# etrigger/Parsip

Measured on AMD Instinct MI355X. Metric: Mcells/sec polygonized, 256^3 grid 32-prim BlobTree, at 1/2/4/8 MI355X, higher is better.
Workload: dtype f32

## Files before the change

parsip_amd/csrc/psgpu_device.h:

```cpp
#pragma once
#include "psgpu_model.h"

namespace psgpu {

typedef const __attribute__((address_space(4))) DevModel* ModelPtr;
typedef const __attribute__((address_space(4))) DevPrim CPrim;
typedef const __attribute__((address_space(4))) DevOp COp;
typedef const __attribute__((address_space(4))) CubeTablesDev* TablePtr;
__device__ __forceinline__ ModelPtr as_const(const DevModel* m) { return (ModelPtr)m; }
__device__ __forceinline__ TablePtr as_const(const CubeTablesDev* t) { return (TablePtr)t; }

__device__ __forceinline__ Instr load_instr(ModelPtr M, int pc) {
    typedef const __attribute__((address_space(4))) uint32_t* CU32;
    const CU32 w = (CU32)(&M->instr[pc]);
    const uint32_t words[3] = {w[0], w[1], w[2]};
    Instr I;
    __builtin_memcpy(&I, words, 12);
    return I;
}

__device__ __forceinline__ float max_ref(float a, float b) { return a > b ? a : b; }
__device__ __forceinline__ float min_ref(float a, float b) { return a < b ? a : b; }
__device__ __forceinline__ float m01(bool c) { return c ? 1.0f : 0.0f; }
__device__ __forceinline__ int lane_id() { return __lane_id(); }
// ... 539 lines not shown
    return (hw & 0xffffu) | (xcc << 16);
}
__device__ __forceinline__ void mpu_ticks_s1(const Params& p, uint32_t w, uint64_t t0) {
    uint64_t* r = p.mpuTicks + 4 * (size_t)w;
    r[0] = t0;
    r[1] = stamp_now();
    r[2] = 0ull;
    r[3] = (uint64_t)wave_hw_id();
}
__device__ __forceinline__ void mpu_ticks_s2(const Params& p, uint32_t m) {
    const uint64_t t = stamp_now();
    const uint32_t hw = wave_hw_id();
    if (lane_id() == 0) {
        uint64_t* r = p.mpuTicks + 4 * (size_t)(m - p.mpuBegin);
        atomicMax(reinterpret_cast<unsigned long long*>(r + 2), (unsigned long long)t);
        reinterpret_cast<uint32_t*>(r + 3)[1] = hw;
    }
}
#define PSGPU_STAMPED(K, ITEM, CALL)                                             \
    {                                                                             \
        const uint64_t t0_ = (p.stamps || p.spans) ? psgpu::stamp_now() : 0ull;  \
        uint32_t item_ = blockIdx.x * (blockDim.x >> 6) + (threadIdx.x >> 6);     \
        CALL;                                                                     \
        if (K == 1 && p.mpuTicks && ITEM != 0xffffffffu) psgpu::mpu_ticks_s2(p, ITEM); \
        if (p.stamps) psgpu::stamp_end(p, K, t0_, ITEM);                          \
        if (p.spans) psgpu::span_end(p, K, t0_);                                  \
    }

__device__ __forceinline__ void mpu_origin(const Params& p, uint32_t m, float o[3]) {
    uint32_t k, jk;
    const uint32_t i = div_by(m, p.dims[2] * p.dims[1], p.divMagic[1], &jk);
    const uint32_t j = div_by(jk, p.dims[2], p.divMagic[0], &k);
    o[0] = p.lo[0] + (float)i * p.side;
    o[1] = p.lo[1] + (float)j * p.side;
    o[2] = p.lo[2] + (float)k * p.side;
}

__device__ __forceinline__ uint32_t wave_sum(uint32_t v) { return lane_value(wave_incl_scan(v), 63); }


__device__ __forceinline__ uint32_t front_tag(const Params& p) { return p.ctr->epoch + 1u; }

__device__ __forceinline__ void stamp_live_word(const Params& p, bool on, const CullMask& cm, uint64_t above) {
    if (on && p.stamps && lane_id() == 0) {
        const uint32_t w = blockIdx.x * (blockDim.x >> 6) + (threadIdx.x >> 6);
        if (w < p.stampCap)
            p.stamps[3 * (size_t)kNumStampKernels * p.stampCap + 8 * (size_t)w + 7] =
                (uint64_t)(128 - __popcll(cm.lo) - __popcll(cm.hi)) | above;
    }
}

__device__ __forceinline__ BoundBox octant_box(const Params& p, const float o[3], int c) {
    BoundBox B;
#pragma unroll
    for (int i = 0; i < 4; ++i) {
        B.xs[i] = o[0] + (float)(4 * (c & 1) + i) * p.cs;
        B.ys[i] = o[1] + (float)(4 * ((c >> 1) & 1) + i) * p.cs;
        B.zs[i] = o[2] + (float)(4 * (c >> 2) + i) * p.cs;
    }
    const float hx = 0.5f * (B.xs[3] - B.xs[0]), hy = 0.5f * (B.ys[3] - B.ys[0]), hz = 0.5f * (B.zs[3] - B.zs[0]);
    B.cx = 0.5f * (B.xs[0] + B.xs[3]);
    B.cy = 0.5f * (B.ys[0] + B.ys[3]);
    B.cz = 0.5f * (B.zs[0] + B.zs[3]);
    B.h = __builtin_amdgcn_sqrtf(hx * hx + hy * hy + hz * hz) * 1.0001f + 1e-4f;
    float mag = 0.0f;
#pragma unroll
    for (int a = 0; a < 3; ++a)
        mag = fmaxf(mag, fmaxf(fabsf(p.lo[a]), fabsf(p.lo[a] + (float)p.dims[a] * p.side)));
    B.hx = B.hy = B.hz = (1.5f * p.cs + 2.4e-7f * (mag + p.side)) * 1.0001f + 1e-4f;
    return B;
}

__device__ __forceinline__ uint32_t proven_mask(bool ok, float lo, float hi, uint32_t flags8) {
    const uint64_t bOut = ballot(ok && hi < 0.5f), bIn = ballot(ok && lo >= 0.5f);
    uint32_t proven8 = 0;
#pragma unroll
    for (int q = 0; q < 8; ++q) {
        const bool all = ((bOut >> (8 * q)) & 0xffull) == 0xffull || ((bIn >> (8 * q)) & 0xffull) == 0xffull;
        proven8 |= (all ? 1u : 0u) << q;
    }
    return proven8 & flags8;
}

__device__ __forceinline__ CullMask queue_masks(const Params& p, const CullLanes& cl, const float o[3],
                                                uint32_t queue8, uint32_t mOf, int lane) {
    CullMask mine{0ull, 0ull};
    if (!p.cull) return mine;
    const float eg = 7.0f * p.cs + 0.001f;
    ModelPtr Mo = as_const(p.model);
    const uint32_t nOps = p.opInside ? Mo->ctOps : 0u;
    float bl[2][3], bh[2][3];
#pragma unroll
    for (int h = 0; h < 2; ++h) {
        const uint32_t k = 64u * h + (uint32_t)lane;
#pragma unroll
        for (int a = 0; a < 3; ++a) {
            bl[h][a] = k < nOps ? p.model->ops[k].lo[a] : 1.0f;
            bh[h][a] = k < nOps ? p.model->ops[k].hi[a] : -1.0f;
        }
    }
    for (uint32_t qm = queue8; qm != 0u; qm &= qm - 1u) {
        const int q = __builtin_ctz(qm);
        const float ox = __int_as_float(__builtin_amdgcn_readlane(__float_as_int(o[0]), 8 * q));
        const float oy = __int_as_float(__builtin_amdgcn_readlane(__float_as_int(o[1]), 8 * q));
        const float oz = __int_as_float(__builtin_amdgcn_readlane(__float_as_int(o[2]), 8 * q));
        CullMask g = cull_mask_from(cl, ox, oy, oz, ox + eg, oy + eg, oz + eg);
        if (nOps != 0u) g.inLo = ballot((uint32_t)lane < nOps && op_inside_box(bl[0], bh[0], ox, oy, oz, p.cs));
        if (nOps > 64u)
            g.inHi = ballot(64u + (uint32_t)lane < nOps && op_inside_box(bl[1], bh[1], ox, oy, oz, p.cs));
        const uint32_t wq = lane_value(mOf, q) - p.mpuBegin;
        if (lane == 0) {
            p.mpuMasks[4 * wq] = g.lo;
            p.mpuMasks[4 * wq + 1] = g.hi;
            p.mpuMasks[4 * wq + 2] = g.inLo;
            p.mpuMasks[4 * wq + 3] = g.inHi;
        }
        if (lane == q) mine = g;
    }
    return mine;
}

struct QueueEntry {
    uint32_t m;
    CullMask cm;

    template <bool FRONT, class T>
    static __device__ __forceinline__ void put(T* at, T v) {
        if constexpr (FRONT) __hip_atomic_store(at, v, __ATOMIC_RELAXED, __HIP_MEMORY_SCOPE_AGENT);
        else *at = v;
    }
    template <bool FRONT, class T>
    static __device__ __forceinline__ T get(T* at) {
        if constexpr (FRONT) return __hip_atomic_load(at, __ATOMIC_RELAXED, __HIP_MEMORY_SCOPE_AGENT);
        else return *at;
    }
    template <bool FRONT>
    __device__ __forceinline__ void store(const Params& p, uint32_t slotq) const {
        put<FRONT>(&p.pq[slotq], m);
        if (p.cull) {
            put<FRONT>(&p.pqMask[4 * slotq], cm.lo);
            put<FRONT>(&p.pqMask[4 * slotq + 1], cm.hi);
            put<FRONT>(&p.pqMask[4 * slotq + 2], cm.inLo);
            put<FRONT>(&p.pqMask[4 * slotq + 3], cm.inHi);
        }
    }
    static __device__ __forceinline__ void publish(const Params& p, uint32_t slotq, bool mine) {
        asm volatile("s_waitcnt vmcnt(0)" ::: "memory");
        if (mine) put<true>(&p.fqReady[slotq], front_tag(p));
    }
    template <bool FRONT>
    static __device__ __forceinline__ QueueEntry load(const Params& p, ModelPtr M, uint32_t slotq) {
        QueueEntry e{uniform(get<FRONT>(&p.pq[slotq])), CullMask{0ull, 0ull}};
        if (p.cull) {
            e.cm.lo = uniform64(get<FRONT>(&p.pqMask[4 * slotq]));
            e.cm.hi = uniform64(get<FRONT>(&p.pqMask[4 * slotq + 1]));
            e.cm.inLo = uniform64(get<FRONT>(&p.pqMask[4 * slotq + 2]));
            if (!FRONT || M->ctOps > 64u) e.cm.inHi = uniform64(get<FRONT>(&p.pqMask[4 * slotq + 3]));
        }
        return e;
    }
};

template <class EV, int SPLIT = 1, bool FRONT = false>
__device__ __forceinline__ void precheck_body(const Params& p, float* lds) {
    const int wave = (int)uniform((uint32_t)wave_index());
    const int lane = lane_id();
    const int part = wave % SPLIT;
    const int slot = wave / SPLIT;
    phase_stamp(p, 0, 8192u);
    const uint64_t tick0 = p.mpuTicks ? stamp_now() : 0ull;
    if (blockIdx.x == 0 && threadIdx.x == 0) {
        p.hostCtr->surfaceErr = 0u;
        p.totals[7] = 0u;
    }
    EV ev(as_const(p.model), lds + wave * p.slotsPerLane * 64 + lane);
    CullLanes cl;
    if (p.cull) cl = load_cull_lanes(as_const(p.model));
    const uint32_t W = blockIdx.x * (4u / SPLIT) + (uint32_t)slot;
    uint32_t Wq = W;
    if constexpr (SPLIT == 2) asm volatile("" : "+v"(Wq));
    const uint32_t bzN = p.brickDims[2], byN = p.brickDims[1];
    const uint32_t nBricks = p.brickDims[0] * byN * bzN;
    uint32_t bi, bj, bk;
    bool idle = W >= nBricks;
    if (p.sieve) {
        typedef const __attribute__((address_space(4))) uint64_t* CU64;
        typedef const __attribute__((address_space(4))) uint32_t* CU32;
        const uint64_t e = W < nBricks ? ((CU64)p.liveList)[W] : 0ull;
        idle = W >= *(CU32)&p.ctr->liveBricks;
        bi = (uint32_t)e & 0x1fffffu;
        bj = (uint32_t)(e >> 21) & 0x1fffffu;
        bk = (uint32_t)(e >> 42);
    } else {
        const uint32_t B =
            (idle || p.brickStride == 1u) ? W : (uint32_t)(((uint64_t)W * p.brickStride) % nBricks);
        uint32_t jk;
        bi = p.brickI0 + div_by(B, byN * bzN, p.brickMagic[1], &jk);
        bj = div_by(jk, bzN, p.brickMagic[0], &bk);
    }
    if (SPLIT == 1 && idle) return;
    const uint32_t g = (uint32_t)lane >> 3;
    const uint32_t mi = 2u * bi + ((g >> 2) & 1u);
    const uint32_t mj = 2u * bj + ((g >> 1) & 1u);
    const uint32_t mk = 2u * bk + (g & 1u);
    const uint32_t mg = (mi * p.dims[1] + mj) * p.dims[2] + mk;
    const bool valid = !idle && mi < p.dims[0] && mj < p.dims[1] && mk < p.dims[2] && mg >= p.mpuBegin &&
                       mg - p.mpuBegin < p.mpuCount;
    const uint32_t ci = min(mi, p.dims[0] - 1u), cj = min(mj, p.dims[1] - 1u), ck = min(mk, p.dims[2] - 1u);
    const uint32_t m = valid ? mg : (ci * p.dims[1] + cj) * p.dims[2] + ck;
    const float o[3] = {p.lo[0] + (float)ci * p.side, p.lo[1] + (float)cj * p.side,
                        p.lo[2] + (float)ck * p.side};
    const int c = lane & 7;
    const float X = (float)(c & 1), Y = (float)((c >> 1) & 1), Z = (float)(c >> 2);
    const float px = X * p.side + o[0];
    const float py = Y * p.side + o[1];
    const float pz = Z * p.side + o[2];
    float blo[3], bhi[3];
    brick_box(p.lo, p.side, p.dims, bi, bj, bk, blo, bhi);
    float f = -1.0f;
    CullMask cm{0ull, 0ull};
    if (p.cull) cm = cull_mask_from(cl, blo[0], blo[1], blo[2], bhi[0], bhi[1], bhi[2]);
    if constexpr (SPLIT == 2) {
        __shared__ float sF[4][64];
        float fp = -1.0f;
        if (!(p.debug & 8u) && !idle) {
            if (part == 0) ev.template evaln_part<4, false, 1, 0>(&px, &py, &pz, cm, &fp, nullptr);
            else ev.template evaln_part<4, false, 1, 1>(&px, &py, &pz, cm, &fp, nullptr);
        }
        sF[wave][lane] = fp;
        __syncthreads();
        const float rv = sF[slot * 2][lane], lv = sF[slot * 2 + 1][lane];
        if (!(p.debug & 8u)) ev.template combine<false, 1>(&rv, nullptr, &lv, nullptr, cm, &f, nullptr);
    } else if (!(p.debug & 8u)) {
        f = ev.template eval<4, false>(px, py, pz, cm, nullptr);
    } else if (p.debug & 16u) {
        f = (float)(cm.lo & 1ull) - 1.0f;
    }
    const uint64_t bal = ballot(valid && f > 0.0f);
    phase_stamp(p, 1, 8192u);
    stamp_live_word(p, p.debug & 8192u, cm, (uint64_t)__popcll(bal) << 16);
    uint32_t flags8 = 0;
#pragma unroll
    for (int q = 0; q < 8; ++q) flags8 |= (((bal >> (8 * q)) & 0xffull) != 0ull ? 1u : 0u) << q;
    uint32_t proven8 = 0;
    float lo = 0.0f, hi = 0.0f;
    bool ok = true;
    if ((p.debug & 1024u) && flags8 != 0u) __builtin_amdgcn_s_setprio(2);
    if constexpr (SPLIT == 2) {
        __shared__ float sLo[4][64], sHi[4][64];
        __shared__ uint32_t sOk[4][64];
        const bool doBound = p.bound && flags8 != 0u;
        if (doBound) {
            const BoundBox B = octant_box(p, o, c);
            if (part == 0) ev.template bound_part<0>(B, cm, &lo, &hi, &ok);
            else ev.template bound_part<1>(B, cm, &lo, &hi, &ok);
        }
        sLo[wave][lane] = lo;
        sHi[wave][lane] = hi;
        sOk[wave][lane] = ok ? 1u : 0u;
        __syncthreads();
        if (part != 0) return;
        if (doBound) {
            const int r = slot * 2, l = slot * 2 + 1;
            ok = sOk[r][lane] != 0u && sOk[l][lane] != 0u;
            ev.bound_combine(sLo[r][lane], sHi[r][lane], sLo[l][lane], sHi[l][lane], cm, &lo, &hi);
            proven8 = proven_mask(ok, lo, hi, flags8);
        }
    } else if (p.bound && flags8 != 0u) {
        ev.bound(octant_box(p, o, c), cm, &lo, &hi, &ok);
        proven8 = proven_mask(ok, lo, hi, flags8);
        phase_stamp(p, 2, 8192u);
    }
    const uint32_t queue8 = flags8 & ~proven8;
    const uint32_t mOf = __shfl(m, lane * 8 & 63);
    const bool vOf = __shfl(valid ? 1 : 0, lane * 8 & 63) != 0;
    const bool pass = lane < 8 && ((queue8 >> lane) & 1u);
    if (lane < 8 && vOf) {
        p.passed[mOf - p.mpuBegin] = (uint8_t)(((flags8 >> lane) & 1u) + ((queue8 >> lane) & 1u));
        if (!pass) p.counts[mOf - p.mpuBegin] = 0ull;
        if (p.mpuTicks) mpu_ticks_s1(p, mOf - p.mpuBegin, tick0);
    }
    if (flags8 == 0u) return;
    const uint32_t shard = Wq / (p.pShardCap / 8u);
    if (lane == 1 && proven8 != 0u) atomicAdd(&p.ctr->shard[shard].b, (uint32_t)__popc(proven8));
    if (queue8 == 0u) return;
    const uint32_t qsel = FRONT ? (blockIdx.x & 7u) : shard;
    const uint32_t qbase = FRONT ? qsel * p.fqCap : shard * p.pShardCap;
    uint32_t baseAtomic = 0;
    if (lane == 0) baseAtomic = atomicAdd(&p.ctr->shard[qsel].p, (uint32_t)__popc(queue8));
    const QueueEntry e{mOf, queue_masks(p, cl, o, queue8, mOf, lane)};
    asm volatile("" : "+v"(baseAtomic) : "v"(e.cm.lo));
    const uint32_t base = lane_value(baseAtomic, 0);
    const uint32_t slotq = pass ? qbase + base + (uint32_t)__popc(queue8 & ((1u << lane) - 1u)) : 0u;
    if (pass) e.template store<FRONT>(p, slotq);
    phase_stamp(p, 3, 8192u);
    if constexpr (FRONT) QueueEntry::publish(p, slotq, pass);
}

#ifndef PSGPU_S2_N
#define PSGPU_S2_N 8
#endif
struct MpuLds {
    uint16_t edgeVid[1536];
    uint8_t cfg[344];
    uint16_t firstV[344], firstT[344];
    alignas(8) uint64_t ins[8];
    uint32_t q[2];
};
constexpr int kLdsMpu = (int)((sizeof(MpuLds) + 15) & ~(size_t)15);
static_assert(kLdsMpu == 4864 && __builtin_offsetof(MpuLds, ins) == 4792, "what the host sizes the launch by");
constexpr int kLdsWaveSlots = kMpusPerBlock * kLdsMpu;

__device__ __forceinline__ int find_cell(const uint16_t* first, uint32_t r) {
    int lo = 0;
#pragma unroll
    for (int step = 256; step > 0; step >>= 1) {
        const int mid = lo + step;
        if (mid < 343 && (uint32_t)first[mid] <= r) lo = mid;
    }
    return lo;
}

template <int WPM>
__device__ __forceinline__ void mpu_sync() {
    if (WPM > 1) {
        __syncthreads();
    } else {
        __builtin_amdgcn_fence(__ATOMIC_SEQ_CST, "wavefront");
        __builtin_amdgcn_wave_barrier();
    }
}

__device__ __forceinline__ uint32_t acquire_front(const Params& p, uint32_t q, uint32_t e) {
    const uint32_t slotq = q * p.fqCap + e, live = 0x80000000u;
    if (e >= p.fqCap) return slotq;
    const uint32_t tag = front_tag(p);
    const uint32_t need = p.preBlocks > q ? (p.preBlocks - q + 7u) / 8u : 0u;
    for (uint32_t spins = 0;; ++spins) {
        if (QueueEntry::get<true>(&p.fqReady[slotq]) == tag) return slotq | live;
        if ((spins & 7u) == 7u && QueueEntry::get<true>(&p.ctr->shard[q].s1Done) >= need)
            return slotq | (QueueEntry::get<true>(&p.fqReady[slotq]) == tag ? live : 0u);
        if (spins > ((p.debug & (1u << 27)) ? 8u : (1u << 22))) {
            atomicOr(&p.ctr->error, 4u);
            return slotq;
        }
        __builtin_amdgcn_s_sleep(1);
    }
}

__device__ __forceinline__ uint32_t acquire_queued(const Params& p, const uint32_t* sIncl, uint32_t d,
                                                   uint32_t incl) {
    const uint32_t pshard = (uint32_t)__popcll(ballot(incl <= d));
    const uint32_t pidx = d - (pshard ? sIncl[pshard - 1] : 0u);
    return uniform(pshard * p.pShardCap + pidx);
}

__device__ __forceinline__ auto s2_parts() -> float (*)[8][64] {
    __shared__ float s[4][8][64];
    return s;
}

template <class EV, int SPLIT>
__device__ __forceinline__ uint32_t block_s2_inside_bits(EV& ev, const Params& p, bool live, const float o[3],
                                                         const CullMask& cm, int wave, uint64_t* sIns,
                                                         uint64_t ins[8]) {
    constexpr int NX = 8;
    const int lane = lane_id();
    float fs[NX];
    if (live) {
        const float cs = p.cs;
        const int y = lane >> 3, z = lane & 7;
        const float py = o[1] + (float)y * cs;
        const float pz = o[2] + (float)z * cs;
// ... 895 lines not shown
```

parsip_amd/csrc/psgpu_jit.cpp:

```cpp
#include <hip/hip_runtime.h>
#include <hip/hiprtc.h>

#include <unistd.h>

#include <filesystem>
#include <future>

#include <cstdio>
#include <cstdlib>
#include <cstring>
#include <map>
#include <memory>
#include <mutex>
#include <sstream>
#include <string>
#include <vector>

#include "psgpu_jit.h"
#include "psgpu_model.h"

#include "_psgpu_embed.h"

namespace psgpu {
namespace {
// ... 403 lines not shown
        if (!bound_eligible()) {
            o << "    *lo = 0.0f;\n    *hi = 0.0f;\n    *ok = false;\n  }\n";
            return;
        }
        if (baked) emit_constants();
        if (M.ctOps == 0) {
            o << "    float sl = 0.0f, sh = 0.0f;\n";
            for (uint32_t i = 0; i < M.ctPrims; ++i) {
                const std::string t = bound_prim((int)i);
                o << "    sl = sl + " << t << "l;\n    sh = sh + " << t << "h;\n";
            }
            o << "    *lo = sl;\n    *hi = sh;\n  }\n";
            return;
        }
        emit_bound_op(0, 0);
        o << "    *lo = b0l;\n    *hi = b0h;\n  }\n";
    }
};

constexpr unsigned kBakedNoPacked = 0xf0u;
unsigned packed_fp32_policy(bool baked) {
    unsigned m[2] = {0xffu, kBakedNoPacked};
    if (const char* e = getenv("PSGPU_JIT_NOPK")) {
        unsigned a = 0, b = 0;
        if (sscanf(e, "%x %x", &a, &b) == 2) {
            m[0] = a & 0xffu;
            m[1] = b & 0xffu;
        }
    }
    return m[baked ? 1 : 0];
}

std::string generate_tree_eval(const DevModel& M, bool baked, bool split) {
    Gen g(M, baked);
    std::ostringstream& o = g.o;
    o << "// generated by psgpu_jit.cpp for one BlobTree structure\n";
    o << "#include \"psgpu_device.h\"\nnamespace psgpu {\nstruct TreeEval {\n  ModelPtr M;\n";
    o << "  __device__ TreeEval(ModelPtr m, float*) : M(m) {}\n";
    o << "  template <int GROUP, bool COLOR, int N>\n";
    o << "  __device__ __forceinline__ void evaln(const float* px, const float* py, const float* pz, "
         "const CullMask& cm, float* out, float* colOut) const {\n";
    if (baked) g.emit_constants();
    if (M.ctOps == 0) {
        o << "    float acc[N];\n" << Gen::FN("acc[n] = 0.0f;");
        for (uint32_t i = 0; i < M.ctPrims; ++i) {
            const std::string ce = g.cull_expr((int)i);
            if (ce == "false") {
                o << Gen::FN("acc[n] = acc[n] + " + g.prim_call((int)i) + ";");
            } else {
                o << "    if (!" << ce << ") {\n" << Gen::FN("acc[n] = acc[n] + " + g.prim_call((int)i) + ";")
                  << "    } else {\n" << Gen::FN("acc[n] = acc[n] + 0.0f;") << "    }\n";
            }
        }
        o << Gen::FN("{\n      out[n] = acc[n];\n      if (COLOR) { colOut[3 * n] = " + g.prim(0) +
                     ".col[0]; colOut[3 * n + 1] = " + g.prim(0) + ".col[1]; colOut[3 * n + 2] = " + g.prim(0) +
                     ".col[2]; }\n    }");
    } else {
        for (uint32_t k = 0; k < M.nInstr; ++k)
            if (M.instr[k].kind == kOp && !op_known(M.instr[k].type)) g.trackLast = true;
        if (g.trackLast) o << "    float last[N];\n" << Gen::FN("last[n] = 0.0f;");
        g.zeroSkip = !g.trackLast;
        g.groups = !baked && getenv("PSGPU_JIT_GROUPS") != nullptr;
        g.emit_op(0, 0, "");
        g.groups = false;
        o << Gen::FN(std::string("{\n      out[n] = ") + (g.trackLast ? "last[n]" : "v0[n]") +
                     ";\n      if (COLOR) { colOut[3 * n] = v0c0[n]; colOut[3 * n + 1] = v0c1[n]; colOut[3 * n + 2] = "
                     "v0c2[n]; }\n    }");
    }
    o << "  }\n";
    o << "  template <int GROUP, bool COLOR>\n";
    o << "  __device__ __forceinline__ float eval(float px, float py, float pz, const CullMask& cm, float* colOut) "
         "const {\n    float r;\n    evaln<GROUP, COLOR, 1>(&px, &py, &pz, cm, &r, colOut);\n    return r;\n  }\n";
    g.emit_bound();
    g.emit_split();
    o << "};\n}  // namespace psgpu\n\n";
    const unsigned nopk = packed_fp32_policy(baked);
    static const char* kAttrs[8] = {"PSGPU_PRE_ATTR",  "PSGPU_MPU_ATTR",  "PSGPU_VTX_ATTR",  "PSGPU_FIN_ATTR",
                                    "PSGPU_PRES_ATTR", "PSGPU_MPUS_ATTR", "PSGPU_VTXQ_ATTR", "PSGPU_FINS_ATTR"};
    for (int k = 0; k < 8; ++k)
        o << "#ifndef " << kAttrs[k] << "\n#define " << kAttrs[k]
          << (((nopk >> k) & 1u) ? " __attribute__((target(\"no-packed-fp32-ops\")))" : "") << "\n#endif\n";
    o << "#ifndef PSGPU_FIN_SGPR\n#define PSGPU_FIN_SGPR" << (baked ? "" : " __attribute__((amdgpu_num_sgpr(96)))")
      << "\n#endif\n";
    o << "extern \"C\" __global__ void __launch_bounds__(256) PSGPU_PRE_ATTR jit_precheck(psgpu::Params p) {\n"
         "  extern __shared__ float lds[];\n"
         "  PSGPU_STAMPED(0, item_, psgpu::precheck_body<psgpu::TreeEval>(p, lds));\n}\n";
    o << "extern \"C\" __global__ void __launch_bounds__(256) PSGPU_MPU_ATTR jit_mpu(psgpu::Params p) {\n"
         "  extern __shared__ __attribute__((aligned(16))) unsigned char smem[];\n"
         "  PSGPU_STAMPED(1, item_, psgpu::mpu_body<psgpu::TreeEval>(p, smem, &item_));\n}\n";
    o << "extern \"C\" __global__ void __launch_bounds__(256) PSGPU_MPU_ATTR jit_front(psgpu::Params p) {\n"
         "  extern __shared__ __attribute__((aligned(16))) unsigned char smem[];\n"
         "  psgpu::front_body<psgpu::TreeEval, 1>(p, smem);\n}\n";
    if (split && g.splittable()) {
    o << "extern \"C\" __global__ void __launch_bounds__(256) PSGPU_PRES_ATTR jit_precheck_s(psgpu::Params p) {\n"
         "  extern __shared__ float lds[];\n"
         "  PSGPU_STAMPED(0, item_, (psgpu::precheck_body<psgpu::TreeEval, 2>(p, lds)));\n}\n";
    o << "extern \"C\" __global__ void __launch_bounds__(256) PSGPU_MPUS_ATTR jit_mpu_s(psgpu::Params p) {\n"
         "  extern __shared__ __attribute__((aligned(16))) unsigned char smem[];\n"
         "  PSGPU_STAMPED(1, item_, (psgpu::mpu_body<psgpu::TreeEval, 2>(p, smem, &item_)));\n}\n";
    }
    o << "extern \"C\" __global__ void __launch_bounds__(256) PSGPU_FINS_ATTR jit_surface(psgpu::Params p) {\n"
         "  extern __shared__ __attribute__((aligned(16))) float slds[];\n"
         "  PSGPU_STAMPED(3, item_, (psgpu::surface_body<psgpu::TreeEval>(p, slds)));\n}\n";
    if (split) {
    o << "extern \"C\" __global__ void __launch_bounds__(256) PSGPU_FIN_ATTR jit_surface_w(psgpu::Params p) {\n"
         "  extern __shared__ __attribute__((aligned(16))) float slds[];\n"
         "  PSGPU_STAMPED(3, item_, (psgpu::surface_body<psgpu::TreeEval, 64>(p, slds)));\n}\n";
    if (g.splittable())
    o << "extern \"C\" __global__ void __launch_bounds__(256) PSGPU_MPUS_ATTR jit_front_s(psgpu::Params p) {\n"
         "  extern __shared__ __attribute__((aligned(16))) unsigned char smem[];\n"
         "  psgpu::front_body<psgpu::TreeEval, 2>(p, smem);\n}\n";
    }
    o << "extern \"C\" __global__ void __launch_bounds__(256) PSGPU_VTXQ_ATTR jit_vertex(psgpu::Params p) {\n"
         "  extern __shared__ __attribute__((aligned(16))) float vlds[];\n"
         "  PSGPU_STAMPED(2, item_, (psgpu::vertex_body<psgpu::TreeEval, 16>(p, vlds)));\n}\n";
    o << "extern \"C\" __global__ void __launch_bounds__(256) PSGPU_VTX_ATTR jit_vertex_w(psgpu::Params p) {\n"
         "  extern __shared__ __attribute__((aligned(16))) float vlds[];\n"
         "  PSGPU_STAMPED(2, item_, (psgpu::vertex_body<psgpu::TreeEval, 64>(p, vlds)));\n}\n";
    o << "extern \"C\" __global__ void __launch_bounds__(256) PSGPU_FIN_ATTR PSGPU_FIN_SGPR jit_finish(psgpu::Params p) {\n"
         "  extern __shared__ __attribute__((aligned(16))) float flds[];\n"
         "  PSGPU_STAMPED(3, item_, (psgpu::finish_body<psgpu::TreeEval, 64>(p, flds)));\n}\n";
    o << "extern \"C\" __global__ void __launch_bounds__(256) PSGPU_FINS_ATTR jit_finish_q(psgpu::Params p) {\n"
         "  extern __shared__ __attribute__((aligned(16))) float flds[];\n"
         "  PSGPU_STAMPED(3, item_, (psgpu::finish_body<psgpu::TreeEval, 16>(p, flds)));\n}\n";
    o << "extern \"C\" __global__ void __launch_bounds__(256) PSGPU_FINS_ATTR jit_finish_p(psgpu::Params p) {\n"
         "  extern __shared__ __attribute__((aligned(16))) float flds[];\n"
         "  PSGPU_STAMPED(3, item_, (psgpu::finish_body<psgpu::TreeEval, 32>(p, flds)));\n}\n";
    o << "extern \"C\" __global__ void __launch_bounds__(256) jit_probe(psgpu::Params p, const float* xyz, float* "
         "out, float* colOut, uint32_t n, int mode) {\n"
         "  extern __shared__ __attribute__((aligned(16))) float plds[];\n"
         "  psgpu::probe_body<psgpu::TreeEval>(p, plds, xyz, out, colOut, n, mode);\n}\n";
    return o.str();
}

uint64_t fnv1a(const std::string& s) {
    uint64_t h = 1469598103934665603ull;
    for (unsigned char ch : s) {
        h ^= ch;
        h *= 1099511628211ull;
    }
    return h;
}

std::string cache_dir() {
    const char* d = getenv("PSGPU_JIT_CACHE");
    if (d && *d) return d;
    const char* home = getenv("HOME");
    return std::string(home && *home ? home : "/tmp") + "/.cache/parsip_amd";
}

bool read_file(const std::string& path, std::vector<char>& out) {
    FILE* f = fopen(path.c_str(), "rb");
    if (!f) return false;
    fseek(f, 0, SEEK_END);
    long n = ftell(f);
    fseek(f, 0, SEEK_SET);
    out.resize(n > 0 ? (size_t)n : 0);
    bool ok = n > 0 && fread(out.data(), 1, (size_t)n, f) == (size_t)n;
    fclose(f);
    return ok;
}

void write_file(const std::string& path, const void* data, size_t n) {
    const std::string tmp = path + ".tmp" + std::to_string((unsigned long)getpid());
    FILE* f = fopen(tmp.c_str(), "wb");
    if (!f) return;
    bool ok = fwrite(data, 1, n, f) == n;
    fclose(f);
    if (ok) rename(tmp.c_str(), path.c_str());
    else remove(tmp.c_str());
}

std::string toolchain_id() {
    int maj = 0, min = 0;
    (void)hiprtcVersion(&maj, &min);
    char b[96];
    snprintf(b, sizeof(b), "hiprtc %d.%d | hip %d | %s", maj, min, (int)HIP_VERSION, kJitArch);
// ... 211 lines not shown
```

parsip_amd/csrc/psgpu_model.h:

```cpp
#pragma once
#ifdef __HIPCC_RTC__
typedef unsigned char uint8_t;
typedef signed char int8_t;
typedef unsigned short uint16_t;
typedef unsigned int uint32_t;
typedef int int32_t;
typedef unsigned long long uint64_t;
typedef long long int64_t;
#elif defined(PSGPU_MODEL_NO_HIP)
#include <stdint.h>
#include <string.h>
#include <mutex>
#include <vector>
#else
#include <stdint.h>
#include <string.h>
#include <hip/hip_runtime.h>
#include <mutex>
#include <vector>
#endif
#if defined(__HIPCC__) || defined(__HIPCC_RTC__)
#define PSGPU_HD __host__ __device__
#define PSGPU_HDI __host__ __device__ __forceinline__
#else
// ... 246 lines not shown
                        cull_rcp(n);
    const float support = (n - S.radius) - (reach * 1.0001f + 1e-6f);
    const float gx = __builtin_fmaxf((__builtin_fabsf(dx) - he[0]) - S.boxHalf, 0.0f);
    const float gy = __builtin_fmaxf((__builtin_fabsf(dy) - he[1]) - S.boxHalf, 0.0f);
    const float gz = __builtin_fmaxf((__builtin_fabsf(dz) - he[2]) - S.boxHalf, 0.0f);
    const float gap = cull_sqrt(gx * gx + gy * gy + gz * gz);
    const float d = __builtin_fmaxf(__builtin_fmaxf(sphere, support), gap);
    return d > 0.0f && d * d >= 1.02f && (lineDist - h > S.axisClear);
}

constexpr float kBoundEps = 2e-4f;

template <int TYPE, class PR>
PSGPU_HDI float prim_true_dist(PR& P, float x, float y, float z, float* axisD, float ev[3]) {
    float d2 = 0.0f;
    ev[0] = ev[1] = ev[2] = 0.0f;
    if (TYPE == PSGPU_T_POINT) {
        const float dx = x - P.pos[0], dy = y - P.pos[1], dz = z - P.pos[2];
        ev[0] = __builtin_fabsf(dx); ev[1] = __builtin_fabsf(dy); ev[2] = __builtin_fabsf(dz);
        d2 = dx * dx + dy * dy + dz * dz;
    } else if (TYPE == PSGPU_T_LINE) {
        const float ux = P.dir[0] - P.pos[0], uy = P.dir[1] - P.pos[1], uz = P.dir[2] - P.pos[2];
        const float dx = x - P.pos[0], dy = y - P.pos[1], dz = z - P.pos[2];
        const float t = (dx * ux + dy * uy + dz * uz) / (ux * ux + uy * uy + uz * uz);
        const float ex = dx - t * ux, ey = dy - t * uy, ez = dz - t * uz;
        ev[0] = __builtin_fabsf(ex); ev[1] = __builtin_fabsf(ey); ev[2] = __builtin_fabsf(ez);
        d2 = ex * ex + ey * ey + ez * ez;
    } else if (TYPE == PSGPU_T_CYLINDER) {
        const float px = x - P.pos[0], py = y - P.pos[1], pz = z - P.pos[2];
        float yy = px * P.dir[0] + py * P.dir[1] + pz * P.dir[2];
        const float rr = px * px + py * py + pz * pz - yy * yy;
        const float r = cull_sqrt(rr > 0.0f ? rr : 0.0f);
        *axisD = r;
        const float xx = __builtin_fmaxf(r - P.res[0], 0.0f);
        const float k = xx > 0.0f ? xx * cull_rcp(r) : 0.0f;
        const float ya = yy > 0.0f ? __builtin_fmaxf(yy - P.res[1], 0.0f) : yy;
        ev[0] = __builtin_fabsf(k * (px - yy * P.dir[0]) + ya * P.dir[0]);
        ev[1] = __builtin_fabsf(k * (py - yy * P.dir[1]) + ya * P.dir[1]);
        ev[2] = __builtin_fabsf(k * (pz - yy * P.dir[2]) + ya * P.dir[2]);
        d2 = xx * xx + ya * ya;
    } else if (TYPE == PSGPU_T_CUBE) {
        ev[0] = __builtin_fmaxf(__builtin_fabsf(x - P.pos[0]) - P.res[0], 0.0f);
        ev[1] = __builtin_fmaxf(__builtin_fabsf(y - P.pos[1]) - P.res[0], 0.0f);
        ev[2] = __builtin_fmaxf(__builtin_fabsf(z - P.pos[2]) - P.res[0], 0.0f);
        d2 = ev[0] * ev[0] + ev[1] * ev[1] + ev[2] * ev[2];
    }
    return cull_sqrt(d2);
}

PSGPU_HDI float wyvill_of_dist(float d) {
    const float t = 1.0f - d * d;
    return t > 0.0f ? (t * t) * t : 0.0f;
}

template <int TYPE, class PR>
PSGPU_HDI void prim_interval(PR& P, float cx, float cy, float cz, float h, float hx, float hy, float hz, float* lo,
                             float* hi, bool* ok) {
    float axisD = 1e30f, ev[3];
    const float d = prim_true_dist<TYPE, PR>(P, cx, cy, cz, &axisD, ev);
    if (TYPE == PSGPU_T_CYLINDER) *ok = *ok && (axisD - h > 0.05f);
    const float reach = (hx * ev[0] + hy * ev[1] + hz * ev[2]) * cull_rcp(d);
    float loD = __builtin_fmaxf(d - h, d - reach);
    const float ux = ev[0] + hx, uy = ev[1] + hy, uz = ev[2] + hz;
    const float hiD = __builtin_fminf(d + h, cull_sqrt(ux * ux + uy * uy + uz * uz));
    if (TYPE == PSGPU_T_POINT || TYPE == PSGPU_T_CUBE) {
        const float gx = __builtin_fmaxf(ev[0] - hx, 0.0f);
        const float gy = __builtin_fmaxf(ev[1] - hy, 0.0f);
        const float gz = __builtin_fmaxf(ev[2] - hz, 0.0f);
        loD = __builtin_fmaxf(loD, cull_sqrt(gx * gx + gy * gy + gz * gz));
    }
    *hi = wyvill_of_dist(__builtin_fmaxf(loD, 0.0f)) + kBoundEps;
    *lo = wyvill_of_dist(hiD) - kBoundEps;
}

PSGPU_HDI void brick_box(const float lo[3], float side, const uint32_t dims[3], uint32_t bi, uint32_t bj,
                               uint32_t bk, float blo[3], float bhi[3]) {
    const uint32_t b[3] = {bi, bj, bk};
    for (int a = 0; a < 3; ++a) {
        const uint32_t m0 = 2u * b[a], last = dims[a] - 1u;
        const uint32_t i0 = m0 < last ? m0 : last, i1 = m0 + 1u < last ? m0 + 1u : last;
        blo[a] = lo[a] + (float)i0 * side;
        bhi[a] = side + (lo[a] + (float)i1 * side);
    }
}

PSGPU_HDI uint32_t div_by(uint32_t m, uint32_t d, uint32_t magic, uint32_t* rem) {
#if defined(__HIP_DEVICE_COMPILE__)
    uint32_t q = __umulhi(m, magic);
#else
    uint32_t q = (uint32_t)(((uint64_t)m * magic) >> 32);
#endif
    uint32_t r = m - q * d;
    if (r >= d) { ++q; r -= d; }
    if (r >= d) { ++q; r -= d; }
    *rem = r;
    return q;
}

struct DevModel {
    uint32_t nInstr;
    uint32_t nSlots;
    uint32_t ctPrims;
    uint32_t ctOps;
    uint32_t boundable;
    uint32_t pad[3];
    Instr instr[kMaxInstr];
    DevOp ops[128];
    DevPrim prims[128];
    CullSeg cull[128];
    float zeroCol[128][4];
    uint64_t rootZero[2];
    uint32_t rootZeroValid;
    uint32_t pad2;
};

#ifndef __HIPCC_RTC__
inline bool prim_maybe_culled(const DevPrim& P) {
    return P.type == PSGPU_T_TRIANGLE ||
           (!P.hasMatrix && (P.type == PSGPU_T_POINT || P.type == PSGPU_T_LINE || P.type == PSGPU_T_CYLINDER ||
                             P.type == PSGPU_T_CUBE));
}
inline bool zero_subtree_set(const DevModel& M, int op, uint64_t m[2], int depth = 0) {
    const Instr* I = nullptr;
    for (uint32_t k = 0; k < M.nInstr && !I; ++k)
        if (M.instr[k].kind == kOp && M.instr[k].idx == op) I = &M.instr[k];
    if (!I || depth > 128) return false;
    const int type = I->type, kind = I->childKind;
    auto child = [&](bool isOp, int id) {
        if (isOp) return zero_subtree_set(M, id, m, depth + 1);
        if (id >= 128 || !prim_maybe_culled(M.prims[id])) return false;
        m[id >> 6] |= 1ull << (id & 63);
        return true;
    };
    if (type >= 14 && type <= 18) return child((kind & 2) != 0, I->L) && child((kind & 1) != 0, I->R);
    if (type >= 22 && type <= 25) return child((kind & 2) != 0, I->L);
    return false;
}
inline bool root_zero_set(const DevModel& M, uint64_t m[2]) {
    m[0] = m[1] = 0ull;
    bool ok = true;
    if (M.ctOps == 0) {
        for (uint32_t k = 0; k < M.nInstr; ++k) {
            const uint32_t id = M.instr[k].idx;
            if (M.instr[k].kind != kSumPrim || id >= 128 || !prim_maybe_culled(M.prims[id])) return false;
            m[id >> 6] |= 1ull << (id & 63);
        }
        ok = M.nInstr > 0;
    } else {
        ok = zero_subtree_set(M, 0, m);
    }
    for (int i = 0; ok && i < 128; ++i)
        if (((m[i >> 6] >> (i & 63)) & 1ull) && !(M.cull[i].radius < __builtin_inff())) ok = false;
    return ok;
}
#endif

struct VertexKey {
    uint32_t w;
    uint32_t vidKey;
};
struct VertexPos {
    float scale;
    uint32_t iv;
};
struct TriRec {
    uint32_t a;
// ... 92 lines not shown
```

Baseline: 370,900.

## Refine per-MPU cull masks from brick-live primitives and skip dead bricks

The precheck now culls against the brick box grown by the MPU margin, then derives each queued MPU's cull mask by testing only the primitives still live for the brick, eight per pass. It uses this path only when that takes fewer passes than recomputing a full mask per MPU. It also marks bricks whose root-zero set is fully culled as dead and skips their field evaluation. Op-inside tests for small op counts now handle two MPUs per ballot via bpermute, mask stores move to per-lane writes, and SGPR caps are added to the precheck kernels. The intent is to cut cull and evaluation work in the precheck, at the cost of more complex control flow and reliance on struct fields (rootZero, CullMask with four words, load_cullseg) that the visible code does not show.

Result: no change. 372,400, median of 6 (+0.4%).

```diff
diff --git a/parsip_amd/csrc/psgpu_device.h b/parsip_amd/csrc/psgpu_device.h
--- a/parsip_amd/csrc/psgpu_device.h
+++ b/parsip_amd/csrc/psgpu_device.h
@@ -645,40 +645,107 @@
     return proven8 & flags8;
 }
 
-__device__ __forceinline__ CullMask queue_masks(const Params& p, const CullLanes& cl, const float o[3],
-                                                uint32_t queue8, uint32_t mOf, int lane) {
-    CullMask mine{0ull, 0ull};
+__device__ __forceinline__ CullMask queue_masks(const Params& p, const CullMask& brick,
+                                                const float o[3], uint32_t queue8, uint32_t mOf, int lane) {
+    CullMask mine{0ull, 0ull, 0ull, 0ull};
     if (!p.cull) return mine;
     const float eg = 7.0f * p.cs + 0.001f;
     ModelPtr Mo = as_const(p.model);
     const uint32_t nOps = p.opInside ? Mo->ctOps : 0u;
-    float bl[2][3], bh[2][3];
-#pragma unroll
-    for (int h = 0; h < 2; ++h) {
-        const uint32_t k = 64u * h + (uint32_t)lane;
+    const bool ops2 = nOps != 0u && nOps <= 32u;
+    uint64_t liveLo, liveHi;
+    live_of(brick.lo, brick.hi, Mo->ctPrims, &liveLo, &liveHi);
+    const bool pairs = queue_pair_passes(liveLo, liveHi) < (uint32_t)__popc(queue8);
+    if (pairs) {
+        mine.lo = brick.lo;
+        mine.hi = brick.hi;
+        float c[3], h, he[3];
+        const bool finite = cull_box(o[0], o[1], o[2], o[0] + eg, o[1] + eg, o[2] + eg, c, &h, he);
+        while ((liveLo | liveHi) != 0ull) {
+            const uint64_t pack = live_chunk(&liveLo, &liveHi);
+            const bool upper = (pack & ~(pack >> 1) & 0x4040404040404040ull) != 0ull;
+            const uint32_t idx = (uint32_t)(pack >> (8 * (lane & 7))) & 0xffu;
+            const bool has = idx != 0xffu;
+            const CullSeg S = load_cullseg(Mo, (int)(has ? idx : 0u));
+            const uint64_t bal = ballot(has && finite && cull_one(S, c[0], c[1], c[2], h, he));
+            const uint32_t byte = (uint32_t)(bal >> (8 * (lane & 7))) & 0xffu;
+#pragma unroll
+            for (int s = 0; s < 8; ++s) {
+                const uint32_t is = (uint32_t)(pack >> (8 * s)) & 0xffu;
+                const uint64_t bit = 1ull << (is & 63u);
+                const uint64_t on = (uint64_t)0 - (uint64_t)((byte >> s) & 1u);
+                mine.lo |= on & (is < 64u ? bit : 0ull);
+                if (upper) mine.hi |= on & (is >= 64u && is < 128u ? bit : 0ull);
+            }
+        }
+    }
+    if (ops2) {
+        const uint32_t k = (uint32_t)lane & 31u;
+        float bl[3], bh[3];
 #pragma unroll
         for (int a = 0; a < 3; ++a) {
-            bl[h][a] = k < nOps ? p.model->ops[k].lo[a] : 1.0f;
-            bh[h][a] = k < nOps ? p.model->ops[k].hi[a] : -1.0f;
-        }
-    }
-    for (uint32_t qm = queue8; qm != 0u; qm &= qm - 1u) {
-        const int q = __builtin_ctz(qm);
-        const float ox = __int_as_float(__builtin_amdgcn_readlane(__float_as_int(o[0]), 8 * q));
-        const float oy = __int_as_float(__builtin_amdgcn_readlane(__float_as_int(o[1]), 8 * q));
-        const float oz = __int_as_float(__builtin_amdgcn_readlane(__float_as_int(o[2]), 8 * q));
-        CullMask g = cull_mask_from(cl, ox, oy, oz, ox + eg, oy + eg, oz + eg);
-        if (nOps != 0u) g.inLo = ballot((uint32_t)lane < nOps && op_inside_box(bl[0], bh[0], ox, oy, oz, p.cs));
-        if (nOps > 64u)
-            g.inHi = ballot(64u + (uint32_t)lane < nOps && op_inside_box(bl[1], bh[1], ox, oy, oz, p.cs));
-        const uint32_t wq = lane_value(mOf, q) - p.mpuBegin;
-        if (lane == 0) {
-            p.mpuMasks[4 * wq] = g.lo;
-            p.mpuMasks[4 * wq + 1] = g.hi;
-            p.mpuMasks[4 * wq + 2] = g.inLo;
-            p.mpuMasks[4 * wq + 3] = g.inHi;
-        }
-        if (lane == q) mine = g;
+            bl[a] = k < nOps ? p.model->ops[k].lo[a] : 1.0f;
+            bh[a] = k < nOps ? p.model->ops[k].hi[a] : -1.0f;
+        }
+        for (uint32_t qm = queue8; qm != 0u;) {
+            const int qa = __builtin_ctz(qm);
+            qm &= qm - 1u;
+            const int qb = qm != 0u ? __builtin_ctz(qm) : qa;
+            qm &= qm - 1u;
+            const int from = (lane < 32 ? qa : qb) << 5;
+            const float ox = __int_as_float(__builtin_amdgcn_ds_bpermute(from, __float_as_int(o[0])));
+            const float oy = __int_as_float(__builtin_amdgcn_ds_bpermute(from, __float_as_int(o[1])));
+            const float oz = __int_as_float(__builtin_amdgcn_ds_bpermute(from, __float_as_int(o[2])));
+            const uint64_t in = ballot(k < nOps && op_inside_box(bl, bh, ox, oy, oz, p.cs));
+            if (lane == qa) mine.inLo = in & 0xffffffffull;
+            if (lane == qb && qb != qa) mine.inLo = in >> 32;
+        }
+    }
+    if (!pairs) {
+        const CullLanes cl = load_cull_lanes(Mo);
+        for (uint32_t qm = queue8; qm != 0u; qm &= qm - 1u) {
+            const int q = __builtin_ctz(qm);
+            const float ox = __int_as_float(__builtin_amdgcn_readlane(__float_as_int(o[0]), 8 * q));
+            const float oy = __int_as_float(__builtin_amdgcn_readlane(__float_as_int(o[1]), 8 * q));
+            const float oz = __int_as_float(__builtin_amdgcn_readlane(__float_as_int(o[2]), 8 * q));
+            const CullMask g = cull_mask_from(cl, ox, oy, oz, ox + eg, oy + eg, oz + eg);
+            if (lane == q) {
+                mine.lo = g.lo;
+                mine.hi = g.hi;
+            }
+        }
+    }
+    if (nOps > 32u) {
+        float bl[2][3], bh[2][3];
+#pragma unroll
+        for (int h = 0; h < 2; ++h) {
+            const uint32_t k = 64u * h + (uint32_t)lane;
+#pragma unroll
+            for (int a = 0; a < 3; ++a) {
+                bl[h][a] = k < nOps ? p.model->ops[k].lo[a] : 1.0f;
+                bh[h][a] = k < nOps ? p.model->ops[k].hi[a] : -1.0f;
+            }
+        }
+        for (uint32_t qm = queue8; qm != 0u; qm &= qm - 1u) {
+            const int q = __builtin_ctz(qm);
+            const float ox = __int_as_float(__builtin_amdgcn_readlane(__float_as_int(o[0]), 8 * q));
+            const float oy = __int_as_float(__builtin_amdgcn_readlane(__float_as_int(o[1]), 8 * q));
+            const float oz = __int_as_float(__builtin_amdgcn_readlane(__float_as_int(o[2]), 8 * q));
+            const uint64_t inLo = ballot((uint32_t)lane < nOps && op_inside_box(bl[0], bh[0], ox, oy, oz, p.cs));
+            uint64_t inHi = 0ull;
+            if (nOps > 64u) inHi = ballot(64u + (uint32_t)lane < nOps && op_inside_box(bl[1], bh[1], ox, oy, oz, p.cs));
+            if (lane == q) {
+                mine.inLo = inLo;
+                mine.inHi = inHi;
+            }
+        }
+    }
+    if (lane < 8 && ((queue8 >> lane) & 1u)) {
+        const uint32_t wq = mOf - p.mpuBegin;
+        p.mpuMasks[4 * wq] = mine.lo;
+        p.mpuMasks[4 * wq + 1] = mine.hi;
+        p.mpuMasks[4 * wq + 2] = mine.inLo;
+        p.mpuMasks[4 * wq + 3] = mine.inHi;
     }
     return mine;
 }
@@ -779,21 +846,25 @@
     const float py = Y * p.side + o[1];
     const float pz = Z * p.side + o[2];
     float blo[3], bhi[3];
-    brick_box(p.lo, p.side, p.dims, bi, bj, bk, blo, bhi);
+    brick_box_grown(p.lo, p.side, p.dims, bi, bj, bk, 7.0f * p.cs + 0.001f, blo, bhi);
     float f = -1.0f;
     CullMask cm{0ull, 0ull};
     if (p.cull) cm = cull_mask_from(cl, blo[0], blo[1], blo[2], bhi[0], bhi[1], bhi[2]);
+    ModelPtr Mz = as_const(p.model);
+    const bool dead = p.cull && Mz->rootZeroValid != 0u &&
+                      ((Mz->rootZero[0] & ~cm.lo) | (Mz->rootZero[1] & ~cm.hi)) == 0ull;
     if constexpr (SPLIT == 2) {
         __shared__ float sF[4][64];
         float fp = -1.0f;
-        if (!(p.debug & 8u) && !idle) {
+        if (!(p.debug & 8u) && !idle && !dead) {
             if (part == 0) ev.template evaln_part<4, false, 1, 0>(&px, &py, &pz, cm, &fp, nullptr);
             else ev.template evaln_part<4, false, 1, 1>(&px, &py, &pz, cm, &fp, nullptr);
         }
         sF[wave][lane] = fp;
         __syncthreads();
         const float rv = sF[slot * 2][lane], lv = sF[slot * 2 + 1][lane];
-        if (!(p.debug & 8u)) ev.template combine<false, 1>(&rv, nullptr, &lv, nullptr, cm, &f, nullptr);
+        if (!(p.debug & 8u) && !dead) ev.template combine<false, 1>(&rv, nullptr, &lv, nullptr, cm, &f, nullptr);
+    } else if (dead) {
     } else if (!(p.debug & 8u)) {
         f = ev.template eval<4, false>(px, py, pz, cm, nullptr);
     } else if (p.debug & 16u) {
@@ -851,7 +922,7 @@
     const uint32_t qbase = FRONT ? qsel * p.fqCap : shard * p.pShardCap;
     uint32_t baseAtomic = 0;
     if (lane == 0) baseAtomic = atomicAdd(&p.ctr->shard[qsel].p, (uint32_t)__popc(queue8));
-    const QueueEntry e{mOf, queue_masks(p, cl, o, queue8, mOf, lane)};
+    const QueueEntry e{mOf, queue_masks(p, cm, o, queue8, mOf, lane)};
     asm volatile("" : "+v"(baseAtomic) : "v"(e.cm.lo));
     const uint32_t base = lane_value(baseAtomic, 0);
     const uint32_t slotq = pass ? qbase + base + (uint32_t)__popc(queue8 & ((1u << lane) - 1u)) : 0u;
diff --git a/parsip_amd/csrc/psgpu_jit.cpp b/parsip_amd/csrc/psgpu_jit.cpp
--- a/parsip_amd/csrc/psgpu_jit.cpp
+++ b/parsip_amd/csrc/psgpu_jit.cpp
@@ -509,7 +509,11 @@
           << (((nopk >> k) & 1u) ? " __attribute__((target(\"no-packed-fp32-ops\")))" : "") << "\n#endif\n";
     o << "#ifndef PSGPU_FIN_SGPR\n#define PSGPU_FIN_SGPR" << (baked ? "" : " __attribute__((amdgpu_num_sgpr(96)))")
       << "\n#endif\n";
-    o << "extern \"C\" __global__ void __launch_bounds__(256) PSGPU_PRE_ATTR jit_precheck(psgpu::Params p) {\n"
+    o << "#ifndef PSGPU_PRE_SGPR\n#define PSGPU_PRE_SGPR" << (baked ? "" : " __attribute__((amdgpu_num_sgpr(98)))")
+      << "\n#endif\n";
+    o << "#ifndef PSGPU_PRES_SGPR\n#define PSGPU_PRES_SGPR" << (baked ? "" : " __attribute__((amdgpu_num_sgpr(96)))")
+      << "\n#endif\n";
+    o << "extern \"C\" __global__ void __launch_bounds__(256) PSGPU_PRE_ATTR PSGPU_PRE_SGPR jit_precheck(psgpu::Params p) {\n"
          "  extern __shared__ float lds[];\n"
          "  PSGPU_STAMPED(0, item_, psgpu::precheck_body<psgpu::TreeEval>(p, lds));\n}\n";
     o << "extern \"C\" __global__ void __launch_bounds__(256) PSGPU_MPU_ATTR jit_mpu(psgpu::Params p) {\n"
@@ -519,7 +523,7 @@
          "  extern __shared__ __attribute__((aligned(16))) unsigned char smem[];\n"
          "  psgpu::front_body<psgpu::TreeEval, 1>(p, smem);\n}\n";
     if (split && g.splittable()) {
-    o << "extern \"C\" __global__ void __launch_bounds__(256) PSGPU_PRES_ATTR jit_precheck_s(psgpu::Params p) {\n"
+    o << "extern \"C\" __global__ void __launch_bounds__(256) PSGPU_PRES_ATTR PSGPU_PRES_SGPR jit_precheck_s(psgpu::Params p) {\n"
          "  extern __shared__ float lds[];\n"
          "  PSGPU_STAMPED(0, item_, (psgpu::precheck_body<psgpu::TreeEval, 2>(p, lds)));\n}\n";
     o << "extern \"C\" __global__ void __launch_bounds__(256) PSGPU_MPUS_ATTR jit_mpu_s(psgpu::Params p) {\n"
diff --git a/parsip_amd/csrc/psgpu_model.h b/parsip_amd/csrc/psgpu_model.h
--- a/parsip_amd/csrc/psgpu_model.h
+++ b/parsip_amd/csrc/psgpu_model.h
@@ -352,6 +352,49 @@
         blo[a] = lo[a] + (float)i0 * side;
         bhi[a] = side + (lo[a] + (float)i1 * side);
     }
+}
+
+PSGPU_HDI void brick_box_grown(const float lo[3], float side, const uint32_t dims[3], uint32_t bi, uint32_t bj,
+                               uint32_t bk, float eg, float blo[3], float bhi[3]) {
+    const uint32_t b[3] = {bi, bj, bk};
+    for (int a = 0; a < 3; ++a) {
+        const uint32_t m0 = 2u * b[a], last = dims[a] - 1u;
+        const uint32_t i0 = m0 < last ? m0 : last, i1 = m0 + 1u < last ? m0 + 1u : last;
+        blo[a] = lo[a] + (float)i0 * side;
+        bhi[a] = (lo[a] + (float)i1 * side) + eg;
+    }
+}
+
+PSGPU_HDI void live_of(uint64_t culledLo, uint64_t culledHi, uint32_t ctPrims, uint64_t* lo, uint64_t* hi) {
+    const uint32_t n = ctPrims < 128u ? ctPrims : 128u;
+    *lo = ~culledLo & (n >= 64u ? ~0ull : (1ull << n) - 1ull);
+    *hi = n <= 64u ? 0ull : ~culledHi & (n >= 128u ? ~0ull : (1ull << (n - 64u)) - 1ull);
+}
+PSGPU_HDI uint64_t live_chunk(uint64_t* lo, uint64_t* hi) {
+    uint64_t pack = 0ull;
+    for (int s = 0; s < 8; ++s) {
+        uint64_t idx = 0xffull;
+        if (*lo != 0ull) {
+            idx = (uint64_t)__builtin_ctzll(*lo);
+            *lo &= *lo - 1ull;
+        } else if (*hi != 0ull) {
+            idx = 64ull + (uint64_t)__builtin_ctzll(*hi);
+            *hi &= *hi - 1ull;
+        }
+        pack |= idx << (8 * s);
+    }
+    return pack;
+}
+PSGPU_HDI void live_deposit(uint64_t pack, uint32_t byte, uint64_t* lo, uint64_t* hi) {
+    for (; byte != 0u; byte &= byte - 1u) {
+        const uint32_t idx = (uint32_t)(pack >> (8 * __builtin_ctz(byte))) & 0xffu;
+        const uint64_t bit = 1ull << (idx & 63u);
+        *lo |= idx < 64u ? bit : 0ull;
+        *hi |= idx >= 64u && idx < 128u ? bit : 0ull;
+    }
+}
+PSGPU_HDI uint32_t queue_pair_passes(uint64_t liveLo, uint64_t liveHi) {
+    return (uint32_t)(__builtin_popcountll(liveLo) + __builtin_popcountll(liveHi) + 7) / 8u;
 }
 
 PSGPU_HDI uint32_t div_by(uint32_t m, uint32_t d, uint32_t magic, uint32_t* rem) {
```
